# RoboticExplorationLab/TrajectoryOptimization.jl

Hardware: NVIDIA H100
Metric: ilqr_iterations_per_sec (higher is better)
Workload: dtype f64

## Files before the change

trajectoryoptimization.jl_b200/csrc/capi.cu:

```cuda
#include <cmath>
#include <cstdio>
#include <cstring>
#include <string>
#include <vector>

#include "../../include/trajopt_b200.h"
#include "frag_layout.cuh"
#include "kernels.h"

namespace {

std::string g_create_error;

struct Scratch {
    void* ptr = nullptr;
    size_t bytes = 0;
};

}

struct to_handle {
    DevProblem P{};
    int device = 0;
    cudaStream_t stream = nullptr;
// ... 446 lines not shown
    P.ldab = (mn >= 8 && mn <= 16 && mn + mm + 1 <= 20) ? 20 : ((mn + mm + 1) & ~1);
    std::memcpy(P.params, params, sizeof(params));
    set_default_options(P.opt);
    h->t0 = s->t0;
    const int n = mn, m = mm, N = s->N, B = s->B;

    h->h_costs.resize(s->ncost);
    P.all_diag_cost = 1;
    for (int i = 0; i < s->ncost; i++) {
        int rc = build_cost(h, s->costs[i], n, m, h->h_costs[i]);
        if (rc) return bail(rc);
        if (!h->h_costs[i].diag) P.all_diag_cost = 0;
        if (h->h_costs[i].quat || h->h_costs[i].expr) { P.all_diag_cost = 0; P.dense_riccati = 1; }
    }
    P.lie = s->error_state ? 1 : 0; P.qs = 3; P.ne = P.lie ? n - 1 : n;
    if (P.lie) P.dense_riccati = 1;
    {
        bool diag_costs = true;
        for (const auto& c : h->h_costs) if (!c.diag || c.expr || c.quat) diag_costs = false;
        bool diag_cons = true;
        for (int i = 0; i < s->ncon; i++) if (s->cons[i].kind != TO_CON_GOAL && s->cons[i].kind != TO_CON_BOUND) diag_cons = false;
        P.compact = (P.lie && diag_costs && diag_cons && P.ne == 12 && m == 4) ? 1 : 0;
        const char* nf = getenv("TO_NO_FRAG");
        P.frag = (P.compact && !(nf && atoi(nf) != 0)) ? 1 : 0;
    }
    if (P.dense_riccati && !P.compact) h->overlap = false;
    h->h_cost_index.assign(s->cost_index, s->cost_index + N);
    for (int k = 0; k < N; k++)
        if (h->h_cost_index[k] < 0 || h->h_cost_index[k] >= s->ncost) { h->err = "cost_index out of range"; return bail(TO_EINVAL); }
    h->h_cons.resize(s->ncon);
    P.all_diag_con = 1; P.lambda_len = 0;
    for (int i = 0; i < s->ncon; i++) {
        int rc = build_con(h, s->cons[i], n, m, N, h->h_cons[i]);
        if (rc) return bail(rc);
        h->h_cons[i].offset = P.lambda_len;
        P.lambda_len += (h->h_cons[i].last - h->h_cons[i].first + 1) * h->h_cons[i].p;
        if (h->h_cons[i].kind == CON_GOAL) { h->h_cons[i].goff = P.ngoal; P.ngoal += h->h_cons[i].p; }
        if (!h->h_cons[i].diagonal) P.all_diag_con = 0;
    }
    P.ncost = s->ncost; P.ncon = s->ncon;
    P.max_p_knot = 0; P.max_terms_per_z = 0;
    for (int j = 0; j < n + m; j++) {
        int cnt = 0;
        for (const auto& c : h->h_cons) if (c.diagonal) cnt += (c.row_max[j] >= 0) + (c.kind == CON_BOUND && c.row_min[j] >= 0);
        P.max_terms_per_z = std::max(P.max_terms_per_z, cnt);
    }
    P.max_cons_knot = 0;
    for (int k = 1; k <= N; k++) {
        int pk = 0, nk = 0;
        for (const auto& c : h->h_cons) if (k >= c.first && k <= c.last) { pk += c.p; nk++; }
        P.max_p_knot = std::max(P.max_p_knot, pk);
        P.max_cons_knot = std::max(P.max_cons_knot, nk);
    }
    h->h_mu.assign(s->ncon, P.opt.penalty_initial);
    h->h_dt.assign(s->dt, s->dt + (N - 1));
    h->h_dyn = dyn_tab; h->h_dyn_index = dyn_idx;

    int rc = TO_OK;
    double* d_dt = nullptr; int* d_ci = nullptr;
    P.strideX = (size_t)B * N * n; P.strideU = (size_t)B * (N - 1) * m;
#define ALLOC(ptr, count) if (!rc) rc = dalloc(h, &(ptr), (size_t)(count))
    ALLOC(d_dt, N - 1); ALLOC(d_ci, N);
    DevDyn* d_dyn = nullptr; int* d_dyni = nullptr;
    if (!h->h_dyn.empty()) { ALLOC(d_dyn, h->h_dyn.size()); ALLOC(d_dyni, N - 1); }
    ALLOC(h->d_costs, s->ncost); ALLOC(h->d_cons, std::max(1, s->ncon)); ALLOC(h->d_mu, std::max(1, s->ncon));
    ALLOC(P.x0, (size_t)B * n); ALLOC(P.X, TO_NBUF * P.strideX); ALLOC(P.U, TO_NBUF * P.strideU); ALLOC(P.cur, B);
    ALLOC(P.AB, (size_t)B * (N - 1) * n * P.ldab); ALLOC(P.K, (size_t)B * (N - 1) * P.ne * m); ALLOC(P.d, (size_t)B * (N - 1) * m);
    if (P.dense_riccati) {
        const size_t nme = P.ne + m;
        ALLOC(P.ABe, (size_t)B * (N - 1) * P.ne * nme); ALLOC(P.EG, (size_t)B * N * nme); ALLOC(P.EH, (size_t)B * N * nme * nme);
        if (P.compact) ALLOC(P.EC, (size_t)B * N * TO_EC_LEN);
        if (P.frag) ALLOC(P.REC, (size_t)B * N * TO_REC_LEN);
    }
    ALLOC(P.lambda, (size_t)B * std::max(1, P.lambda_len));
    ALLOC(P.rho, B); ALLOC(P.drho, B); ALLOC(P.dV, 2 * (size_t)B); ALLOC(P.J, B); ALLOC(P.Jc, B); ALLOC(P.alpha, B);
    ALLOC(P.bp_status, B); ALLOC(P.ls_iters, B); ALLOC(P.accepted, B); ALLOC(P.acc1, B);
    if (P.frag) { ALLOC(P.late_list, B); ALLOC(P.late_count, 1); }
    ALLOC(h->d_stageX, P.strideX); ALLOC(h->d_stageU, P.strideU); ALLOC(h->d_viol, B); ALLOC(h->d_merit2, 2);
    ALLOC(h->d_work, 1); ALLOC(h->d_err, 1);
    {
        SolveDev& S = h->solve;
        ALLOC(S.state, B); ALLOC(S.status, B); ALLOC(S.iter, B); ALLOC(S.outer, B); ALLOC(S.inner, B); ALLOC(S.dj_zero, B);
        ALLOC(S.J_prev, B); ALLOC(S.dJ, B); ALLOC(S.grad, B); ALLOC(S.cmax, B); ALLOC(S.n_active, 1);
    }
    if (P.frag) { ALLOC(h->d_fragq, frag_queue_ints(B)); ALLOC(h->d_fragpool, frag_pool_doubles(B, N)); ALLOC(h->d_fragerr, 1); ALLOC(h->d_exptab, 1); }
#undef ALLOC
    if (rc) return bail(rc);
    P.exptab = h->d_exptab;
    P.dyn = d_dyn; P.dyn_index = d_dyni;
    P.dt = d_dt; P.cost_index = d_ci; P.costs = h->d_costs; P.cons = h->d_cons; P.mu = h->d_mu; P.viol = h->d_viol;
    cudaStream_t st = h->stream;
    bool okc = true;
    okc &= cudaMemcpyAsync(d_dt, h->h_dt.data(), sizeof(double) * (N - 1), cudaMemcpyHostToDevice, st) == cudaSuccess;
    okc &= cudaMemcpyAsync(d_ci, h->h_cost_index.data(), sizeof(int) * N, cudaMemcpyHostToDevice, st) == cudaSuccess;
    if (d_dyn) {
        okc &= cudaMemcpyAsync(d_dyn, h->h_dyn.data(), sizeof(DevDyn) * h->h_dyn.size(), cudaMemcpyHostToDevice, st) == cudaSuccess;
        okc &= cudaMemcpyAsync(d_dyni, h->h_dyn_index.data(), sizeof(int) * (N - 1), cudaMemcpyHostToDevice, st) == cudaSuccess;
    }
    okc &= cudaMemsetAsync(P.x0, 0, sizeof(double) * B * n, st) == cudaSuccess;
    okc &= cudaMemsetAsync(P.X, 0xFF, sizeof(double) * TO_NBUF * P.strideX, st) == cudaSuccess;
    okc &= cudaMemsetAsync(P.U, 0, sizeof(double) * TO_NBUF * P.strideU, st) == cudaSuccess;
    okc &= cudaMemsetAsync(P.cur, 0, sizeof(int) * B, st) == cudaSuccess;
    okc &= cudaMemsetAsync(P.AB, 0, sizeof(double) * (size_t)B * (N - 1) * n * P.ldab, st) == cudaSuccess;
    okc &= cudaMemsetAsync(P.K, 0, sizeof(double) * (size_t)B * (N - 1) * P.ne * m, st) == cudaSuccess;
    okc &= cudaMemsetAsync(P.d, 0, sizeof(double) * (size_t)B * (N - 1) * m, st) == cudaSuccess;
    okc &= cudaMemsetAsync(P.lambda, 0, sizeof(double) * (size_t)B * std::max(1, P.lambda_len), st) == cudaSuccess;
// ... 900 lines not shown
```

trajectoryoptimization.jl_b200/csrc/common.cuh:

```cuda
#pragma once
#include <cuda_runtime.h>
#include <cstdlib>
#include <stdint.h>

#define TO_MAXN 16
#define TO_MAXM 8
#define TO_MAXNM (TO_MAXN + TO_MAXM)
#define TO_MAXCON 8
#define TO_MAXP 32
#define TO_MAXPV (2 * TO_MAXNM)
#define TO_CON_A 256
#define TO_EXPR_LEN 128
#define TO_EXPR_CONST 64
#define TO_EC_LEN 40
#define TO_NBUF 9

enum { MODEL_DOUBLE_INTEGRATOR = 0, MODEL_CARTPOLE = 1, MODEL_QUADROTOR = 2, MODEL_ACROBOT = 3, MODEL_EXPR = 4 };
enum { CONE_ZERO = 0, CONE_NEGATIVE_ORTHANT = 1, CONE_SECOND_ORDER = 2, CONE_IDENTITY = 3, CONE_POSITIVE_ORTHANT = 4 };
enum { CON_GOAL = 0, CON_BOUND = 1, CON_LINEAR = 2, CON_CIRCLE = 3, CON_SPHERE = 4, CON_NORM = 5, CON_COLLISION = 6, CON_QUATVEC = 7, CON_EXPR = 8 };

struct DevCost {
    int diag, terminal, zeroH, pad;
    double c;
    double Qd[TO_MAXN], Rd[TO_MAXM];
// ... 53 lines not shown
};

struct DevProblem {
    int model, n, m, N, B;
    int ldab;
    int ncost, ncon, lambda_len;
    int all_diag_cost;
    int all_diag_con;
    int max_p_knot;
    int max_terms_per_z;
    int max_cons_knot;
    int lie, ne, qs, dense_riccati;
    int compact, frag;
    double* EC;
    double* REC;
    const ExpTab* exptab;
    const DevDyn* dyn;
    const int* dyn_index;
    double* ABe;
    double* EG;
    double* EH;
    double params[16];
    DevOptions opt;
    const double* dt;
    const DevCost* costs;
    const int* cost_index;
    const DevCon* cons;
    const double* mu;
    double* x0;
    double* X;
    double* U;
    int* cur;
    double* AB;
    double* K;
    double* d;
    double* lambda;
    double* rho;
    double* drho;
    double* dV;
    double* J;
    double* Jc;
    double* viol;
    double* alpha;
    int* bp_status;
    int* ls_iters;
    int* accepted;
    int* acc1;
    int* late_list;
    int* late_count;
    size_t strideX, strideU;
    const int* active;
    const double* qr;
    const double* goal;
    int ngoal, pad_inst;
};

enum { SOLVE_ACTIVE = 0, SOLVE_WAITING = 1, SOLVE_DONE = 2 };
__host__ __device__ inline bool retired(const DevProblem& P, int b) { return P.active != nullptr && P.active[b] != SOLVE_ACTIVE; }

template <bool INST>
__host__ __device__ __forceinline__ const double* inst_q(const DevProblem& P, int b, int cid) {
    if constexpr (INST) { if (P.qr) return P.qr + ((size_t)b * P.ncost + cid) * (P.n + P.m); }
    return P.costs[cid].q;
}
template <bool INST>
__host__ __device__ __forceinline__ const double* inst_r(const DevProblem& P, int b, int cid) {
    if constexpr (INST) { if (P.qr) return P.qr + ((size_t)b * P.ncost + cid) * (P.n + P.m) + P.n; }
    return P.costs[cid].r;
}
template <bool INST>
__host__ __device__ __forceinline__ const double* goal_values(const DevProblem& P, int b, int ci) {
    if constexpr (INST) { if (P.goal) return P.goal + (size_t)b * P.ngoal + P.cons[ci].goff; }
    return P.cons[ci].a;
}

__host__ __device__ inline const double* traj_X(const DevProblem& P, int buf, int b) { return P.X + buf * P.strideX + (size_t)b * P.N * P.n; }
__host__ __device__ inline const double* traj_U(const DevProblem& P, int buf, int b) { return P.U + buf * P.strideU + (size_t)b * (P.N - 1) * P.m; }
__host__ __device__ inline double* traj_Xw(const DevProblem& P, int buf, int b) { return P.X + buf * P.strideX + (size_t)b * P.N * P.n; }
__host__ __device__ inline double* traj_Uw(const DevProblem& P, int buf, int b) { return P.U + buf * P.strideU + (size_t)b * (P.N - 1) * P.m; }

#define TO_MAXDEV 64
inline int current_device_slot() { int d = 0; cudaGetDevice(&d); return (d >= 0 && d < TO_MAXDEV) ? d : 0; }

__host__ __device__ inline void reg_increase(const DevOptions& o, double& rho, double& drho) {
    drho = fmax(drho * o.bp_reg_increase_factor, o.bp_reg_increase_factor);
    rho = fmax(rho * drho, o.bp_reg_min);
}
__host__ __device__ inline void reg_decrease(const DevOptions& o, double& rho, double& drho) {
    drho = fmin(drho / o.bp_reg_increase_factor, 1.0 / o.bp_reg_increase_factor);
    rho = rho * drho * ((rho * drho > o.bp_reg_min) ? 1.0 : 0.0);
}
```

trajectoryoptimization.jl_b200/csrc/forward.cu:

```cuda
#include <cstdlib>
#include "costcon.cuh"
#include "kernels.h"
#include "models.cuh"

namespace {

constexpr int FWD_MAX_COST = 4;
constexpr int FWD_MAX_N = 512;
constexpr int FWD_THREADS = 32;

struct FwdCon {
    int kind, first, last, p, offset;
    unsigned mask_max, mask_min;
    int ubox;
    double mu, inv2mu;
    int row_max[TO_MAXNM], row_min[TO_MAXNM];
    double a[TO_MAXNM], b[TO_MAXNM];
};
struct FwdCost {
    double Qd[TO_MAXN], Rd[TO_MAXM], q[TO_MAXN], r[TO_MAXM], c;
};
struct alignas(16) FwdTab {
    int ncon, ncost_cached, pad0, pad1;
    FwdCon con[TO_MAXCON];
    FwdCost cost[FWD_MAX_COST];
    double dt[FWD_MAX_N];
    int cost_index[FWD_MAX_N];
    int lam_off[FWD_MAX_N][2];
    int lam_cnt[FWD_MAX_N][2];
};

__device__ inline void load_tables(const DevProblem& P, FwdTab& tab) {
    const int t = threadIdx.x, T = blockDim.x;
    if (t == 0) { tab.ncon = P.ncon; tab.ncost_cached = P.ncost <= FWD_MAX_COST ? P.ncost : 0; }
    for (int ci = 0; ci < P.ncon; ci++) {
        const DevCon& c = P.cons[ci];
        FwdCon& f = tab.con[ci];
        if (t == 0) {
            f.kind = c.kind; f.first = c.first; f.last = c.last; f.p = c.p; f.offset = c.offset;
            f.mu = P.mu[ci]; f.inv2mu = 1.0 / (2.0 * P.mu[ci]);
            unsigned mx = 0, mn = 0;
            for (int j = 0; j < TO_MAXNM; j++) { if (c.row_max[j] >= 0) mx |= 1u << j; if (c.row_min[j] >= 0) mn |= 1u << j; }
            f.mask_max = mx; f.mask_min = mn;
            const unsigned ubits = ((1u << P.m) - 1u) << P.n;
            f.ubox = (c.kind == CON_BOUND && mx == ubits && mn == ubits) ? 1 : 0;
        }
        for (int j = t; j < TO_MAXNM; j += T) {
            f.row_max[j] = c.row_max[j]; f.row_min[j] = c.row_min[j];
            f.a[j] = c.a[j]; f.b[j] = c.b[j];
        }
    }
    if (P.ncost <= FWD_MAX_COST)
        for (int ci = 0; ci < P.ncost; ci++) {
            const DevCost& c = P.costs[ci];
            FwdCost& f = tab.cost[ci];
            for (int j = t; j < TO_MAXN; j += T) { f.Qd[j] = c.Qd[j]; f.q[j] = c.q[j]; }
            for (int j = t; j < TO_MAXM; j += T) { f.Rd[j] = c.Rd[j]; f.r[j] = c.r[j]; }
            if (t == 0) f.c = c.c;
        }
    for (int k = t; k < P.N && k < FWD_MAX_N; k += T) {
        tab.dt[k] = (k < P.N - 1) ? P.dt[k] : 0.0; tab.cost_index[k] = P.cost_index[k];
        int ns = 0;
        tab.lam_cnt[k][0] = tab.lam_cnt[k][1] = 0; tab.lam_off[k][0] = tab.lam_off[k][1] = 0;
        for (int ci = 0; ci < P.ncon; ci++) {
            const DevCon& c = P.cons[ci];
            if (k + 1 < c.first || k + 1 > c.last) continue;
            if (ns < 2) { tab.lam_off[k][ns] = c.offset + (k + 1 - c.first) * c.p; tab.lam_cnt[k][ns] = c.p; }
            ns++;
        }
    }
    __syncthreads();
}

__device__ __forceinline__ void cp_async8(double* smem_dst, const double* gsrc) {
    asm volatile("cp.async.ca.shared.global [%0], [%1], 8;" ::"r"((uint32_t)__cvta_generic_to_shared(smem_dst)), "l"(gsrc) : "memory");
}
__device__ __forceinline__ void cp_async16(double* smem_dst, const double* gsrc) {
    asm volatile("cp.async.cg.shared.global [%0], [%1], 16;" ::"r"((uint32_t)__cvta_generic_to_shared(smem_dst)), "l"(gsrc) : "memory");
}
__device__ __forceinline__ void cp_async_commit() { asm volatile("cp.async.commit_group;" ::: "memory"); }
#ifndef TO_FWD_STAGES
#define TO_FWD_STAGES 2
#endif
constexpr int FWD_STAGES = TO_FWD_STAGES;
template <int NPEND> __device__ __forceinline__ void cp_async_wait() { asm volatile("cp.async.wait_group %0;" ::"n"(NPEND) : "memory"); }

template <int n, int m, int IPB, int NE = n>
struct Stage {
    static constexpr int KSLOTS = NE * m;
    static constexpr bool K16 = (KSLOTS % 2) == 0;
    static constexpr int OFF_D = KSLOTS, OFF_U = OFF_D + m, OFF_X = OFF_U + m, OFF_L = OFF_X + n;
    static constexpr int LAM_SLOTS = 2 * (n + m);
    static constexpr int NSLOT = OFF_L + LAM_SLOTS;
    static constexpr int DOUBLES = NSLOT * IPB;
    __device__ static __forceinline__ int kidx(int e, int g) { return K16 ? ((e >> 1) * IPB + g) * 2 + (e & 1) : e * IPB + g; }
    __device__ static __forceinline__ int sidx(int slot, int g) { return slot * IPB + g; }
};

template <int n, int m, int IPB, int G, int NE>
__device__ __forceinline__ void prefetch_knot(double* base, int g, int l, int k, const double* Kg, const double* dg, const double* X,
                                              const double* U, const double* lam_b, const FwdTab& tab, int N) {
    using S = Stage<n, m, IPB, NE>;
    if (k < N - 1) {
        const double* Kk = Kg + (size_t)k * NE * m;
        if (S::K16) {
#pragma unroll
            for (int c = 0; c < (S::KSLOTS / 2 + G - 1) / G; c++) {
                const int cc = c * G + l;
                if (cc < S::KSLOTS / 2) cp_async16(base + S::kidx(2 * cc, g), Kk + 2 * cc);
            }
        } else {
#pragma unroll
            for (int c = 0; c < (S::KSLOTS + G - 1) / G; c++) {
                const int cc = c * G + l;
                if (cc < S::KSLOTS) cp_async8(base + S::kidx(cc, g), Kk + cc);
            }
        }
#pragma unroll
        for (int c = 0; c < (2 * m + n + G - 1) / G; c++) {
            const int s = c * G + l;
            if (s < m) cp_async8(base + S::sidx(S::OFF_D + s, g), dg + (size_t)k * m + s);
            else if (s < 2 * m) cp_async8(base + S::sidx(S::OFF_U + s - m, g), U + (size_t)k * m + (s - m));
            else if (s < 2 * m + n) cp_async8(base + S::sidx(S::OFF_X + s - 2 * m, g), X + (size_t)k * n + (s - 2 * m));
        }
    }
    {
        const int c0 = tab.lam_cnt[k][0], c1 = tab.lam_cnt[k][1];
        const double* l0 = lam_b + tab.lam_off[k][0];
        const double* l1 = lam_b + tab.lam_off[k][1];
        for (int i = l; i < c0; i += G) cp_async8(base + S::sidx(S::OFF_L + i, g), l0 + i);
        for (int i = l; i < c1; i += G) cp_async8(base + S::sidx(S::OFF_L + c0 + i, g), l1 + i);
    }
}

template <int MODEL, int IPB, int G, bool LIE, bool INST>
__device__ __forceinline__ double rollout_fast(const DevProblem& P, const FwdTab& tab, double* stage, int b, int g, int l, unsigned gmask,
                                               double alpha, int cbuf, bool& ok, double& viol) {
    constexpr int n = ModelDims<MODEL>::n, m = ModelDims<MODEL>::m, NE = LIE ? n - 1 : n;
    using S = Stage<n, m, IPB, NE>;
    const int N = P.N, buf = P.cur[b];
    const double* X = traj_X(P, buf, b);
    const double* U = traj_U(P, buf, b);
    double* Xc = traj_Xw(P, cbuf, b);
    double* Uc = traj_Uw(P, cbuf, b);
    const double* Kg = P.K + (size_t)b * (N - 1) * NE * m;
    const double* dg = P.d + (size_t)b * (N - 1) * m;
    const double* lam_b = P.lambda + (size_t)b * P.lambda_len;
    double x[n], u[m], xn[n];
    double J = 0.0;
    ok = true; viol = 0.0;
#pragma unroll
    for (int i = 0; i < n; i++) x[i] = P.x0[(size_t)b * n + i];
    constexpr int D = FWD_STAGES - 1;
#pragma unroll
    for (int j = 0; j < D; j++) {
        if (j < N) prefetch_knot<n, m, IPB, G, NE>(stage + j * S::DOUBLES, g, l, j, Kg, dg, X, U, lam_b, tab, N);
        cp_async_commit();
    }
    int sb = 0, sp = D;
    for (int k = 0; k < N; k++) {
        const bool last = (k == N - 1);
        __syncwarp(gmask);
        if (k + D < N) prefetch_knot<n, m, IPB, G, NE>(stage + sp * S::DOUBLES, g, l, k + D, Kg, dg, X, U, lam_b, tab, N);
        cp_async_commit();
        cp_async_wait<D>();
        __syncwarp(gmask);
        const double* st = stage + sb * S::DOUBLES;
        sb = (sb + 1 == FWD_STAGES) ? 0 : sb + 1; sp = (sp + 1 == FWD_STAGES) ? 0 : sp + 1;
        if (!last) {
#pragma unroll
            for (int a = 0; a < m; a++) u[a] = fma(alpha, st[S::sidx(S::OFF_D + a, g)], st[S::sidx(S::OFF_U + a, g)]);
            double dxe[NE];
            if constexpr (LIE) {
                double xr[n];
#pragma unroll
                for (int i = 0; i < n; i++) xr[i] = st[S::sidx(S::OFF_X + i, g)];
                state_diff(true, n, 3, x, xr, dxe);
            } else {
// ... 64 lines not shown
                double a = 0.0, l2 = 0.0;
                if (c.kind == CON_GOAL) {
                    const unsigned mk = c.mask_max;
                    const double* ga = c.a;
                    if constexpr (INST) ga = goal_values<true>(P, b, ci);
#pragma unroll
                    for (int i = 0; i < n; i++) {
                        if (mk & (1u << i)) {
                            const int row = c.row_max[i];
                            const double lm = st[S::sidx(lo + row, g)];
                            const double cv = x[i] - ga[row];
                            const double lp = fma(-mu, cv, lm);
                            a = fma(lp, lp, a); l2 = fma(lm, lm, l2); viol = fmax(viol, fabs(cv));
                        }
                    }
                } else if (c.ubox) {
#pragma unroll
                    for (int i = 0; i < m; i++) {
                        const double lu = st[S::sidx(lo + i, g)], ll = st[S::sidx(lo + m + i, g)];
                        const double cu = u[i] - c.a[n + i], cl = c.b[n + i] - u[i];
                        const double pu = fmin(0.0, fma(-mu, cu, lu)), pl = fmin(0.0, fma(-mu, cl, ll));
                        a = fma(pu, pu, a); a = fma(pl, pl, a); l2 = fma(lu, lu, l2); l2 = fma(ll, ll, l2);
                        viol = fmax(viol, fmax(cu, cl));
                    }
                } else {
                    const unsigned mx = c.mask_max, mn = c.mask_min;
                    if ((mx | mn) & ((1u << n) - 1u)) {
#pragma unroll
                        for (int i = 0; i < n; i++) {
                            if (mx & (1u << i)) { const double lm = st[S::sidx(lo + c.row_max[i], g)]; const double cv = x[i] - c.a[i]; const double lp = fmin(0.0, fma(-mu, cv, lm)); a = fma(lp, lp, a); l2 = fma(lm, lm, l2); viol = fmax(viol, cv); }
                            if (mn & (1u << i)) { const double lm = st[S::sidx(lo + c.row_min[i], g)]; const double cv = c.b[i] - x[i]; const double lp = fmin(0.0, fma(-mu, cv, lm)); a = fma(lp, lp, a); l2 = fma(lm, lm, l2); viol = fmax(viol, cv); }
                        }
                    }
#pragma unroll
                    for (int i = 0; i < m; i++) {
                        if (mx & (1u << (n + i))) { const double lm = st[S::sidx(lo + c.row_max[n + i], g)]; const double cv = u[i] - c.a[n + i]; const double lp = fmin(0.0, fma(-mu, cv, lm)); a = fma(lp, lp, a); l2 = fma(lm, lm, l2); viol = fmax(viol, cv); }
                        if (mn & (1u << (n + i))) { const double lm = st[S::sidx(lo + c.row_min[n + i], g)]; const double cv = c.b[n + i] - u[i]; const double lp = fmin(0.0, fma(-mu, cv, lm)); a = fma(lp, lp, a); l2 = fma(lm, lm, l2); viol = fmax(viol, cv); }
                    }
                }
                J = fma(a - l2, c.inv2mu, J);
                slot += c.p;
            }
        }
        if (!last) {
            rk4_step<MODEL, double>(model_params<MODEL>(P, k), x, u, tab.dt[k], xn);
#pragma unroll
            for (int i = 0; i < n; i++) { x[i] = xn[i]; if (!(fabs(xn[i]) <= P.opt.max_state_value)) ok = false; }
        }
    }
    cp_async_wait<0>();
    return J;
}

template <int MODEL, bool LIE, bool INST>
__device__ __forceinline__ double rollout_generic(const DevProblem& P, int b, double alpha, int cbuf, bool& ok, double& viol) {
    constexpr int n = ModelDims<MODEL>::n, m = ModelDims<MODEL>::m, NE = LIE ? n - 1 : n;
    const int N = P.N, buf = P.cur[b];
    const double* X = traj_X(P, buf, b);
    const double* U = traj_U(P, buf, b);
    double* Xc = traj_Xw(P, cbuf, b);
    double* Uc = traj_Uw(P, cbuf, b);
    const double* Kg = P.K + (size_t)b * (N - 1) * NE * m;
    const double* dg = P.d + (size_t)b * (N - 1) * m;
    const double* lam_b = P.lambda + (size_t)b * P.lambda_len;
    double x[n], u[m], xn[n];
    double J = 0.0;
    ok = true; viol = 0.0;
#pragma unroll
    for (int i = 0; i < n; i++) x[i] = P.x0[(size_t)b * n + i];
    for (int k = 0; k < N; k++) {
        const bool last = (k == N - 1);
        if (!last) {
#pragma unroll
            for (int a = 0; a < m; a++) u[a] = fma(alpha, dg[(size_t)k * m + a], U[(size_t)k * m + a]);
            double dxe[NE], xr[n];
#pragma unroll
            for (int i = 0; i < n; i++) xr[i] = X[(size_t)k * n + i];
            state_diff(LIE, n, 3, x, xr, dxe);
#pragma unroll
            for (int i = 0; i < NE; i++) {
                const double dx = dxe[i];
#pragma unroll
                for (int a = 0; a < m; a++) u[a] = fma(Kg[(size_t)k * NE * m + i * m + a], dx, u[a]);
            }
#pragma unroll
            for (int a = 0; a < m; a++) if (!(fabs(u[a]) <= P.opt.max_control_value)) ok = false;
        } else {
#pragma unroll
            for (int a = 0; a < m; a++) u[a] = 0.0;
        }
#pragma unroll
        for (int i = 0; i < n; i++) Xc[(size_t)k * n + i] = x[i];
        if (!last) {
#pragma unroll
            for (int a = 0; a < m; a++) Uc[(size_t)k * m + a] = u[a];
        }
        const int cid = P.cost_index[k];
        J += cost_value(P.costs[cid], inst_q<INST>(P, b, cid), inst_r<INST>(P, b, cid), n, m, x, u, !last);
        J += al_knot_penalty<INST>(P, k + 1, x, u, lam_b, viol, b);
        if (!last) {
            rk4_step<MODEL, double>(model_params<MODEL>(P, k), x, u, P.dt[k], xn);
#pragma unroll
            for (int i = 0; i < n; i++) { x[i] = xn[i]; if (!(fabs(xn[i]) <= P.opt.max_state_value)) ok = false; }
            if (!ok) break;
        }
    }
    return J;
}

__device__ __forceinline__ bool ls_accept(const DevProblem& P, double J, double J_prev, double alpha, double dV1, double dV2, bool ok) {
    if (!ok) return false;
    const double expected = -alpha * (dV1 + alpha * dV2);
    const double z = expected > 0.0 ? (J_prev - J) / expected : -1.0;
    return (z > P.opt.ls_lower && z <= P.opt.ls_upper) || (J < J_prev);
}

extern __shared__ __align__(16) unsigned char fwd_smem[];

template <int MODEL, int G, bool FAST, int LANES, bool LIE, bool INST>
__global__ void __launch_bounds__(FWD_THREADS) k_linesearch(const DevProblem P, int trial0, int first_pass, int final_pass) {
    constexpr int n = ModelDims<MODEL>::n, m = ModelDims<MODEL>::m, NE = LIE ? n - 1 : n;
    constexpr int IPB = LANES / G;
    using S = Stage<n, m, IPB, NE>;
    FwdTab* tab = reinterpret_cast<FwdTab*>(fwd_smem);
    double* stage = reinterpret_cast<double*>(fwd_smem + sizeof(FwdTab));
    const int g = (threadIdx.x % LANES) / G, l = threadIdx.x % G;
    int b = blockIdx.x * IPB + g;
    if (!first_pass && P.late_list) b = (b < *P.late_count) ? P.late_list[b] : P.B;
    const unsigned gmask = (G == 32) ? 0xffffffffu : (((1u << G) - 1u) << (g * G));
    const bool valid = b < P.B && threadIdx.x < LANES && !retired(P, b);
    const int status = valid ? P.bp_status[b] : -1;
    const int was_accepted = (valid && !first_pass) ? P.accepted[b] : 0;
    const bool work = valid && status >= 0 && !was_accepted && trial0 <= P.opt.ls_iters;
    const unsigned any = __ballot_sync(0xffffffffu, work);
    if (FAST && any) load_tables(P, *tab);
    if (!valid) return;
    bool accepted = was_accepted != 0;
    if (work) {
        const int trial = trial0 + l;
        const double alpha = ldexp(1.0, -trial);
        const int cbuf = (P.cur[b] + 1 + l) % TO_NBUF;
        bool ok = false;
        double J, viol = 0.0;
        if (FAST) J = rollout_fast<MODEL, IPB, G, LIE, INST>(P, *tab, stage, b, g, l, gmask, alpha, cbuf, ok, viol);
        else J = rollout_generic<MODEL, LIE, INST>(P, b, alpha, cbuf, ok, viol);
        const bool good = (trial <= P.opt.ls_iters) && ls_accept(P, J, P.J[b], alpha, P.dV[2 * b], P.dV[2 * b + 1], ok);
        const unsigned votes = __ballot_sync(gmask, good) & gmask;
        if (votes) {
            const int win = __ffs(votes) - 1 - g * G;
            if (l == win) {
                P.cur[b] = cbuf; P.J[b] = J; P.viol[b] = viol; P.alpha[b] = alpha; P.ls_iters[b] = trial + 1; P.accepted[b] = 1;
            }
            accepted = true;
        }
    }
    if (l == 0 && first_pass) {
        P.acc1[b] = accepted ? 1 : 0;
        if (!accepted && P.late_list) P.late_list[atomicAdd(P.late_count, 1)] = b;
    }
    if (l == 0 && !accepted) {
        if (first_pass) P.accepted[b] = 0;
        if (status < 0) { P.alpha[b] = 0.0; P.ls_iters[b] = 0; }
        else if (final_pass) {
            double rho = P.rho[b], drho = P.drho[b];
            reg_increase(P.opt, rho, drho);
            rho += P.opt.bp_reg_fp;
            P.rho[b] = rho; P.drho[b] = drho;
            P.alpha[b] = 0.0; P.ls_iters[b] = P.opt.ls_iters + 1;
        }
    }
    (void)sizeof(S);
}

template <int MODEL, int G, bool FAST, int LANES, bool LIE = false, bool INST = false>
cudaError_t launch_pass_l(const DevProblem& P, int trial0, int first_pass, int final_pass, cudaStream_t s) {
    constexpr int n = ModelDims<MODEL>::n, m = ModelDims<MODEL>::m, NE = LIE ? n - 1 : n;
    constexpr int IPB = LANES / G;
    const int blocks = (P.B + IPB - 1) / IPB;
    const size_t smem = FAST ? sizeof(FwdTab) + (size_t)FWD_STAGES * Stage<n, m, IPB, NE>::DOUBLES * sizeof(double) : 0;
    auto kern = k_linesearch<MODEL, G, FAST, LANES, LIE, INST>;
    static bool configured[TO_MAXDEV] = {false};
    const int dev = current_device_slot();
    if (!configured[dev] && smem > 48 * 1024) {
        cudaError_t e = cudaFuncSetAttribute(kern, cudaFuncAttributeMaxDynamicSharedMemorySize, (int)smem);
        if (e != cudaSuccess) return e;
    }
    configured[dev] = true;
    kern<<<blocks, FWD_THREADS, smem, s>>>(P, trial0, first_pass, final_pass);
    return cudaGetLastError();
}

template <int MODEL, int G, bool FAST, bool INST>
cudaError_t launch_pass_i(const DevProblem& P, int trial0, int first_pass, int final_pass, cudaStream_t s) {
    const int lanes = first_pass ? 16 : (P.late_list ? 16 : 32);
    if constexpr (MODEL == MODEL_QUADROTOR) {
        if (P.lie) {
            if (G <= 16 && lanes == 16) return launch_pass_l<MODEL, G, FAST, (G <= 16 ? 16 : 32), true, INST>(P, trial0, first_pass, final_pass, s);
            return launch_pass_l<MODEL, G, FAST, 32, true, INST>(P, trial0, first_pass, final_pass, s);
        }
    }
    if (G <= 16 && lanes == 16) return launch_pass_l<MODEL, G, FAST, (G <= 16 ? 16 : 32), false, INST>(P, trial0, first_pass, final_pass, s);
    return launch_pass_l<MODEL, G, FAST, 32, false, INST>(P, trial0, first_pass, final_pass, s);
}

template <int MODEL, int G, bool FAST>
cudaError_t launch_pass(const DevProblem& P, int trial0, int first_pass, int final_pass, cudaStream_t s) {
    if (P.qr) return launch_pass_i<MODEL, G, FAST, true>(P, trial0, first_pass, final_pass, s);
    return launch_pass_i<MODEL, G, FAST, false>(P, trial0, first_pass, final_pass, s);
}

bool fast_path(const DevProblem& P) {
    return P.all_diag_cost && P.all_diag_con && P.N <= FWD_MAX_N && P.max_p_knot <= 2 * (P.n + P.m) && P.max_cons_knot <= 2;
}

}

cudaError_t launch_forward(const DevProblem& P, cudaStream_t s) {
    cudaError_t e = cudaErrorNotSupported;
    const int final_pass = P.opt.ls_iters < 4;
    if (P.late_list) { e = cudaMemsetAsync(P.late_count, 0, sizeof(int), s); if (e != cudaSuccess) return e; e = cudaErrorNotSupported; }
    if (fast_path(P)) { TO_DISPATCH_MODEL(P.model, P.m, (e = launch_pass<MODEL, 4, true>(P, 0, 1, final_pass, s))); }
    else { TO_DISPATCH_MODEL(P.model, P.m, (e = launch_pass<MODEL, 4, false>(P, 0, 1, final_pass, s))); }
    return e;
}

cudaError_t launch_ladder(const DevProblem& P, cudaStream_t s) {
    cudaError_t e = cudaSuccess;
    for (int trial0 = 4; trial0 <= P.opt.ls_iters && e == cudaSuccess; trial0 += 8) {
        const int final_pass = trial0 + 8 > P.opt.ls_iters;
        if (fast_path(P)) { TO_DISPATCH_MODEL(P.model, P.m, (e = launch_pass<MODEL, 8, true>(P, trial0, 0, final_pass, s))); }
        else { TO_DISPATCH_MODEL(P.model, P.m, (e = launch_pass<MODEL, 8, false>(P, trial0, 0, final_pass, s))); }
    }
    return e;
}

cudaError_t launch_accept(const DevProblem& P, cudaStream_t s) { return cudaSuccess; }
```

Before: 2.635 million.

## Add compact line-search rollout path for uniform diagonal cost and box constraints

```diff
diff --git a/profiles/linesearch_ab.py b/profiles/linesearch_ab.py
--- /dev/null
+++ b/profiles/linesearch_ab.py
@@ -0,0 +1,75 @@
+#!/usr/bin/env python3
+import argparse, json, os, subprocess, sys, tempfile
+
+import numpy as np
+
+ROOT = os.path.dirname(os.path.dirname(os.path.abspath(__file__)))
+DEFAULT = os.path.join(ROOT, "trajectoryoptimization.jl_b200", "libtrajopt_b200.so")
+VARIANT = os.path.join(ROOT, "trajectoryoptimization.jl_b200", "variants", "lib_fwd_loop.so")
+
+
+def card():
+    q = subprocess.run(["nvidia-smi", "--query-gpu=name,power.limit,clocks.max.sm", "--format=csv,noheader"], capture_output=True, text=True)
+    return q.stdout.strip().splitlines()[0] if q.returncode == 0 and q.stdout.strip() else "unknown"
+
+
+def bench(lib, workload, dump):
+    env = dict(os.environ, LIBTRAJOPT_B200=lib)
+    out = subprocess.run([sys.executable, os.path.join(ROOT, "bench.py"), "--gpus", "1", "--steps", "20", "--warmup", "3", "--workload", workload,
+                          "--no-cpu-baseline", "--dump-outputs", dump], capture_output=True, text=True, env=env, cwd=ROOT)
+    line = [l for l in out.stdout.splitlines() if l.startswith("{")]
+    if out.returncode or not line:
+        raise SystemExit(f"bench.py failed on {lib}:\n{out.stderr[-2000:]}")
+    d = json.loads(line[-1])
+    ph = d["roofline"]["phase_ms"]
+    return dict(step=d["ms_per_step"], F=ph["forward"], L=ph["ladder"], C1E1=ph["cost_expansion"] + ph["expand"],
+                E2C2=ph["late_expansion"], R=ph["backward"], phases=ph)
+
+
+def main():
+    ap = argparse.ArgumentParser()
+    ap.add_argument("--reps", type=int, default=3)
+    ap.add_argument("--workload", default="quadrotor")
+    ap.add_argument("--out", default=None)
+    ap.add_argument("--lib", action="append", default=[], metavar="NAME=PATH", help="further libraries to alternate with the two")
+    args = ap.parse_args()
+    tmp = tempfile.mkdtemp(prefix="linesearch_ab_")
+    variant = VARIANT
+    if not os.path.exists(variant):
+        subprocess.run(["bash", os.path.join(ROOT, "profiles", "scripts", "build_variant.sh"), "fwd_loop", "forward.cu", "-DTO_FWD_COMPACT=0"],
+                       check=True, env=dict(os.environ, VARIANT_DIR=tmp), stdout=subprocess.DEVNULL)
+        variant = os.path.join(tmp, "lib_fwd_loop.so")
+    print(f"card: {card()}  workload: {args.workload}", flush=True)
+    libs = {"rollout_fast (-DTO_FWD_COMPACT=0)": variant, "rollout_compact (default)": DEFAULT}
+    libs.update(dict(kv.split("=", 1) for kv in args.lib))
+    runs = {name: [] for name in libs}
+    dumps = []
+    for r in range(args.reps):
+        for name, lib in libs.items():
+            d = os.path.join(tmp, f"dump_{len(dumps)}")
+            res = bench(lib, args.workload, d)
+            runs[name].append(res); dumps.append((name, d))
+            print(f"  {name:36s} step {res['step']:.4f}  F {res['F']:.4f}  L {res['L']:.4f}  C1+E1 {res['C1E1']:.4f}  "
+                  f"E2/C2 {res['E2C2']:.4f}  R {res['R']:.4f}", flush=True)
+    ref_name, ref = dumps[0]
+    identical = True
+    for name, d in dumps[1:]:
+        for f in sorted(os.listdir(ref)):
+            a, b = np.load(os.path.join(ref, f)), np.load(os.path.join(d, f))
+            if a.shape != b.shape or not np.array_equal(a.view(np.uint8), b.view(np.uint8)):
+                identical = False
+                print(f"  DUMP DIFFERS: {f} of {name} against {ref_name}")
+    print(f"dumps bit-identical across all {len(dumps)} runs: {identical}")
+    for name, rs in runs.items():
+        rng = lambda k: f"{min(x[k] for x in rs):.3f}-{max(x[k] for x in rs):.3f}"
+        print(f"{name:36s} step {rng('step')}  F {rng('F')}  L {rng('L')}  C1+E1 {rng('C1E1')}  E2/C2 {rng('E2C2')}  R {rng('R')}")
+    fa, fb = runs["rollout_fast (-DTO_FWD_COMPACT=0)"], runs["rollout_compact (default)"]
+    print(f"every default run faster than every variant run: {max(x['step'] for x in fb) < min(x['step'] for x in fa)}")
+    if args.out:
+        with open(args.out, "w") as fh:
+            json.dump(dict(card=card(), runs=runs, identical=identical), fh, indent=1)
+    sys.exit(0 if identical else 1)
+
+
+if __name__ == "__main__":
+    main()
diff --git a/trajectoryoptimization.jl_b200/csrc/capi.cu b/trajectoryoptimization.jl_b200/csrc/capi.cu
--- a/trajectoryoptimization.jl_b200/csrc/capi.cu
+++ b/trajectoryoptimization.jl_b200/csrc/capi.cu
@@ -522,6 +522,21 @@
         P.max_p_knot = std::max(P.max_p_knot, pk);
         P.max_cons_knot = std::max(P.max_cons_knot, nk);
     }
+    {
+        bool cls = N >= 2 && P.all_diag_cost && P.all_diag_con;
+        for (int k = 1; k < N - 1; k++) if (h->h_cost_index[k] != h->h_cost_index[0]) cls = false;
+        int nbox = 0, ngc = 0;
+        for (const auto& c : h->h_cons) {
+            if (c.kind == CON_BOUND) {
+                bool ubox = c.first == 1 && c.last == N - 1 && c.p == 2 * m;
+                for (int j = 0; j < n + m; j++) if ((c.row_max[j] >= 0) != (j >= n) || (c.row_min[j] >= 0) != (j >= n)) ubox = false;
+                cls = cls && ubox; nbox++;
+            } else if (c.kind == CON_GOAL) {
+                cls = cls && c.first == N && c.last == N; ngc++;
+            } else cls = false;
+        }
+        P.fwd_compact = (cls && nbox <= 1 && ngc <= 1) ? 1 : 0;
+    }
     h->h_mu.assign(s->ncon, P.opt.penalty_initial);
     h->h_dt.assign(s->dt, s->dt + (N - 1));
     h->h_dyn = dyn_tab; h->h_dyn_index = dyn_idx;
diff --git a/trajectoryoptimization.jl_b200/csrc/common.cuh b/trajectoryoptimization.jl_b200/csrc/common.cuh
--- a/trajectoryoptimization.jl_b200/csrc/common.cuh
+++ b/trajectoryoptimization.jl_b200/csrc/common.cuh
@@ -129,7 +129,8 @@
     const int* active;
     const double* qr;
     const double* goal;
-    int ngoal, pad_inst;
+    int ngoal;
+    int fwd_compact;
 };
 
 enum { SOLVE_ACTIVE = 0, SOLVE_WAITING = 1, SOLVE_DONE = 2 };
diff --git a/trajectoryoptimization.jl_b200/csrc/forward.cu b/trajectoryoptimization.jl_b200/csrc/forward.cu
--- a/trajectoryoptimization.jl_b200/csrc/forward.cu
+++ b/trajectoryoptimization.jl_b200/csrc/forward.cu
@@ -1,4 +1,5 @@
 #include <cstdlib>
+#include <type_traits>
 #include "costcon.cuh"
 #include "kernels.h"
 #include "models.cuh"
@@ -72,6 +73,50 @@
     __syncthreads();
 }
 
+struct alignas(16) FwdCompactTab {
+    double2 sx[TO_MAXN];
+    double2 su[TO_MAXM];
+    double2 box[TO_MAXM];
+    double sc, mu, inv2mu, pad0;
+    int cid, tcid, box_off, box_p;
+    int goal_ci, goal_off, goal_p, pad1;
+    FwdCost term;
+    FwdCon goal;
+    double dt[FWD_MAX_N];
+};
+
+__device__ inline void load_compact_tables(const DevProblem& P, FwdCompactTab& tab) {
+    const int t = threadIdx.x, T = blockDim.x;
+    const int cid = P.cost_index[0], tcid = P.cost_index[P.N - 1];
+    const DevCost& c = P.costs[cid];
+    const DevCost& ct = P.costs[tcid];
+    for (int j = t; j < TO_MAXN; j += T) { tab.sx[j] = make_double2(c.Qd[j], c.q[j]); tab.term.Qd[j] = ct.Qd[j]; tab.term.q[j] = ct.q[j]; }
+    for (int j = t; j < TO_MAXM; j += T) tab.su[j] = make_double2(c.Rd[j], c.r[j]);
+    if (t == 0) {
+        tab.sc = c.c; tab.term.c = ct.c; tab.cid = cid; tab.tcid = tcid;
+        tab.box_off = tab.box_p = 0; tab.goal_ci = -1; tab.goal_off = tab.goal_p = 0;
+    }
+    for (int ci = 0; ci < P.ncon; ci++) {
+        const DevCon& k = P.cons[ci];
+        if (k.kind == CON_BOUND) {
+            for (int j = t; j < P.m; j += T) tab.box[j] = make_double2(k.a[P.n + j], k.b[P.n + j]);
+            if (t == 0) { tab.box_off = k.offset; tab.box_p = k.p; tab.mu = P.mu[ci]; tab.inv2mu = 1.0 / (2.0 * P.mu[ci]); }
+        } else {
+            FwdCon& f = tab.goal;
+            if (t == 0) {
+                tab.goal_ci = ci; tab.goal_off = k.offset; tab.goal_p = k.p;
+                f.mu = P.mu[ci]; f.inv2mu = 1.0 / (2.0 * P.mu[ci]);
+                unsigned mx = 0;
+                for (int j = 0; j < TO_MAXNM; j++) if (k.row_max[j] >= 0) mx |= 1u << j;
+                f.mask_max = mx;
+            }
+            for (int j = t; j < TO_MAXNM; j += T) { f.row_max[j] = k.row_max[j]; f.a[j] = k.a[j]; }
+        }
+    }
+    for (int k = t; k < P.N - 1; k += T) tab.dt[k] = P.dt[k];
+    __syncthreads();
+}
+
 __device__ __forceinline__ void cp_async8(double* smem_dst, const double* gsrc) {
     asm volatile("cp.async.ca.shared.global [%0], [%1], 8;" ::"r"((uint32_t)__cvta_generic_to_shared(smem_dst)), "l"(gsrc) : "memory");
 }
@@ -83,6 +128,7 @@
 #define TO_FWD_STAGES 2
 #endif
 constexpr int FWD_STAGES = TO_FWD_STAGES;
+constexpr int FWD_OKNOTS = 4;
 template <int NPEND> __device__ __forceinline__ void cp_async_wait() { asm volatile("cp.async.wait_group %0;" ::"n"(NPEND) : "memory"); }
 
 template <int n, int m, int IPB, int NE = n>
@@ -98,8 +144,8 @@
 };
 
 template <int n, int m, int IPB, int G, int NE>
-__device__ __forceinline__ void prefetch_knot(double* base, int g, int l, int k, const double* Kg, const double* dg, const double* X,
-                                              const double* U, const double* lam_b, const FwdTab& tab, int N) {
+__device__ __forceinline__ void prefetch_operands(double* base, int g, int l, int k, const double* Kg, const double* dg, const double* X,
+                                                  const double* U, int N) {
     using S = Stage<n, m, IPB, NE>;
     if (k < N - 1) {
         const double* Kk = Kg + (size_t)k * NE * m;
@@ -124,6 +170,13 @@
             else if (s < 2 * m + n) cp_async8(base + S::sidx(S::OFF_X + s - 2 * m, g), X + (size_t)k * n + (s - 2 * m));
         }
     }
+}
+
+template <int n, int m, int IPB, int G, int NE>
+__device__ __forceinline__ void prefetch_knot(double* base, int g, int l, int k, const double* Kg, const double* dg, const double* X,
+                                              const double* U, const double* lam_b, const FwdTab& tab, int N) {
+    using S = Stage<n, m, IPB, NE>;
+    prefetch_operands<n, m, IPB, G, NE>(base, g, l, k, Kg, dg, X, U, N);
     {
         const int c0 = tab.lam_cnt[k][0], c1 = tab.lam_cnt[k][1];
         const double* l0 = lam_b + tab.lam_off[k][0];
@@ -294,6 +347,171 @@
     return J;
 }
 
+template <int MODEL, int IPB, int G, bool LIE, bool INST>
+__device__ __forceinline__ double rollout_compact(const DevProblem& P, const FwdCompactTab& tab, double* stage, double* ost, int b, int g,
+                                                  int l, unsigned gmask, double alpha, int cbuf, bool& ok, double& viol) {
+    constexpr int n = ModelDims<MODEL>::n, m = ModelDims<MODEL>::m, NE = LIE ? n - 1 : n;
+    using S = Stage<n, m, IPB, NE>;
+    const int N = P.N, buf = P.cur[b];
+    const double* X = traj_X(P, buf, b);
+    const double* U = traj_U(P, buf, b);
+    double* Xc = traj_Xw(P, cbuf, b);
+    const double* Kg = P.K + (size_t)b * (N - 1) * NE * m;
+    const double* dg = P.d + (size_t)b * (N - 1) * m;
+    const double* lam_b = P.lambda + (size_t)b * P.lambda_len;
+    constexpr int OX = FWD_OKNOTS * n, OL = FWD_OKNOTS * (n + m);
+    double* myx = ost + l * OL;
+    double* myu = myx + OX;
+    const double* cq = INST ? inst_q<true>(P, b, tab.cid) : nullptr;
+    const double* cr = INST ? inst_r<true>(P, b, tab.cid) : nullptr;
+    const bool box = tab.box_p != 0;
+    double x[n], u[m];
+    double J = 0.0;
+    ok = true; viol = 0.0;
+#pragma unroll
+    for (int i = 0; i < n; i++) x[i] = P.x0[(size_t)b * n + i];
+    constexpr int D = FWD_STAGES - 1;
+    auto prefetch = [&](double* base, int k) {
+        prefetch_operands<n, m, IPB, G, NE>(base, g, l, k, Kg, dg, X, U, N);
+        const bool stg = k < N - 1;
+        const int cnt = stg ? tab.box_p : tab.goal_p;
+        const double* src = lam_b + (stg ? tab.box_off + k * tab.box_p : tab.goal_off);
+        for (int i = l; i < cnt; i += G) cp_async8(base + S::sidx(S::OFF_L + i, g), src + i);
+    };
+#pragma unroll
+    for (int j = 0; j < D; j++) {
+        if (j < N) prefetch(stage + j * S::DOUBLES, j);
+        cp_async_commit();
+    }
+    int sb = 0, sp = D;
+    auto next_stage = [&](int k) -> const double* {
+        __syncwarp(gmask);
+        if (k + D < N) prefetch(stage + sp * S::DOUBLES, k + D);
+        cp_async_commit();
+        cp_async_wait<D>();
+        __syncwarp(gmask);
+        const double* st = stage + sb * S::DOUBLES;
+        sb = (sb + 1 == FWD_STAGES) ? 0 : sb + 1; sp = (sp + 1 == FWD_STAGES) ? 0 : sp + 1;
+        return st;
+    };
+    auto knot = [&](int k, double* x) {
+        const double* st = next_stage(k);
+#pragma unroll
+        for (int a = 0; a < m; a++) u[a] = fma(alpha, st[S::sidx(S::OFF_D + a, g)], st[S::sidx(S::OFF_U + a, g)]);
+        double dxe[NE];
+        if constexpr (LIE) {
+            double xr[n];
+#pragma unroll
+            for (int i = 0; i < n; i++) xr[i] = st[S::sidx(S::OFF_X + i, g)];
+            state_diff(true, n, 3, x, xr, dxe);
+        } else {
+#pragma unroll
+            for (int i = 0; i < n; i++) dxe[i] = x[i] - st[S::sidx(S::OFF_X + i, g)];
+        }
+#pragma unroll
+        for (int i = 0; i < NE; i++) {
+            const double dx = dxe[i];
+            if (S::K16 && (m % 2 == 0)) {
+#pragma unroll
+                for (int a = 0; a < m; a += 2) {
+                    const double2 kv = *reinterpret_cast<const double2*>(&st[S::kidx(i * m + a, g)]);
+                    u[a] = fma(kv.x, dx, u[a]);
+                    u[a + 1] = fma(kv.y, dx, u[a + 1]);
+                }
+            } else {
+#pragma unroll
+                for (int a = 0; a < m; a++) u[a] = fma(st[S::kidx(i * m + a, g)], dx, u[a]);
+            }
+        }
+#pragma unroll
+        for (int a = 0; a < m; a++) if (!(fabs(u[a]) <= P.opt.max_control_value)) ok = false;
+        const int kk = k % FWD_OKNOTS;
+#pragma unroll
+        for (int i = 0; i < n; i++) myx[kk * n + i] = x[i];
+#pragma unroll
+        for (int a = 0; a < m; a++) myu[kk * m + a] = u[a];
+        if (kk == FWD_OKNOTS - 1 || k == N - 2) {
+            __syncwarp(gmask);
+            const int k0 = k - kk, nx = (kk + 1) * n, nu = (kk + 1) * m;
+            for (int j = 0; j < G; j++) {
+                const int cb = (buf + 1 + j) % TO_NBUF;
+                double* xd = traj_Xw(P, cb, b) + (size_t)k0 * n;
+                double* ud = traj_Uw(P, cb, b) + (size_t)k0 * m;
+                const double* xs = ost + j * OL;
+                for (int e = l; e < nx; e += G) xd[e] = xs[e];
+                for (int e = l; e < nu; e += G) ud[e] = xs[OX + e];
+            }
+        }
+        {
+            double a2 = 0.0, l1 = 0.0;
+#pragma unroll
+            for (int i = 0; i < n; i++) { const double2 c = tab.sx[i]; a2 = fma(c.x * x[i], x[i], a2); l1 = fma(INST ? cq[i] : c.y, x[i], l1); }
+#pragma unroll
+            for (int i = 0; i < m; i++) { const double2 c = tab.su[i]; a2 = fma(c.x * u[i], u[i], a2); l1 = fma(INST ? cr[i] : c.y, u[i], l1); }
+            J += fma(0.5, a2, l1) + tab.sc;
+        }
+        if (box) {
+            const double mu = tab.mu;
+            double a = 0.0, l2 = 0.0;
+#pragma unroll
+            for (int i = 0; i < m; i++) {
+                const double lu = st[S::sidx(S::OFF_L + i, g)], ll = st[S::sidx(S::OFF_L + m + i, g)];
+                const double2 bx = tab.box[i];
+                const double cu = u[i] - bx.x, cl = bx.y - u[i];
+                const double vu = fma(-mu, cu, lu), vl = fma(-mu, cl, ll);
+                const double pu = vu < 0.0 ? vu : 0.0, pl = vl < 0.0 ? vl : 0.0;
+                a = fma(pu, pu, a); a = fma(pl, pl, a); l2 = fma(lu, lu, l2); l2 = fma(ll, ll, l2);
+                const double t = cu > cl ? cu : cl;
+                viol = t > viol ? t : viol;
+            }
+            J = fma(a - l2, tab.inv2mu, J);
+        }
+        if constexpr (MODEL == MODEL_EXPR_42) {
+            double xn[n];
+            rk4_step<MODEL, double>(model_params<MODEL>(P, k), x, u, tab.dt[k], xn);
+#pragma unroll
+            for (int i = 0; i < n; i++) x[i] = xn[i];
+        } else {
+            rk4_step<MODEL, double>(model_params<MODEL>(P, k), x, u, tab.dt[k], x);
+        }
+#pragma unroll
+        for (int i = 0; i < n; i++) if (!(fabs(x[i]) <= P.opt.max_state_value)) ok = false;
+    };
+#pragma unroll 1
+    for (int k = 0; k < N - 1; k++) knot(k, x);
+    {
+        const double* st = next_stage(N - 1);
+#pragma unroll
+        for (int i = 0; i < n; i++) Xc[(size_t)(N - 1) * n + i] = x[i];
+        const double* tq = INST ? inst_q<true>(P, b, tab.tcid) : tab.term.q;
+        double a2 = 0.0, l1 = 0.0;
+#pragma unroll
+        for (int i = 0; i < n; i++) { a2 = fma(tab.term.Qd[i] * x[i], x[i], a2); l1 = fma(tq[i], x[i], l1); }
+        J += fma(0.5, a2, l1) + tab.term.c;
+        if (tab.goal_ci >= 0) {
+            const FwdCon& c = tab.goal;
+            const double mu = c.mu;
+            double a = 0.0, l2 = 0.0;
+            const unsigned mk = c.mask_max;
+            const double* ga = c.a;
+            if constexpr (INST) ga = goal_values<true>(P, b, tab.goal_ci);
+#pragma unroll
+            for (int i = 0; i < n; i++) {
+                if (mk & (1u << i)) {
+                    const int row = c.row_max[i];
+                    const double lm = st[S::sidx(S::OFF_L + row, g)];
+                    const double cv = x[i] - ga[row];
+                    const double lp = fma(-mu, cv, lm);
+                    a = fma(lp, lp, a); l2 = fma(lm, lm, l2); viol = fmax(viol, fabs(cv));
+                }
+            }
+            J = fma(a - l2, c.inv2mu, J);
+        }
+    }
+    cp_async_wait<0>();
+    return J;
+}
+
 template <int MODEL, bool LIE, bool INST>
 __device__ __forceinline__ double rollout_generic(const DevProblem& P, int b, double alpha, int cbuf, bool& ok, double& viol) {
     constexpr int n = ModelDims<MODEL>::n, m = ModelDims<MODEL>::m, NE = LIE ? n - 1 : n;
@@ -359,13 +577,20 @@
 
 extern __shared__ __align__(16) unsigned char fwd_smem[];
 
-template <int MODEL, int G, bool FAST, int LANES, bool LIE, bool INST>
-__global__ void __launch_bounds__(FWD_THREADS) k_linesearch(const DevProblem P, int trial0, int first_pass, int final_pass) {
+enum { FWD_GENERIC = 0, FWD_FAST = 1, FWD_COMPACT = 2 };
+#ifndef TO_FWD_COMPACT
+#define TO_FWD_COMPACT 1
+#endif
+
+template <int MODEL, int G, int PATH, int LANES, bool LIE, bool INST>
+__device__ __forceinline__ void linesearch_pass(const DevProblem& P, int trial0, int first_pass, int final_pass) {
     constexpr int n = ModelDims<MODEL>::n, m = ModelDims<MODEL>::m, NE = LIE ? n - 1 : n;
+    constexpr bool FAST = PATH != FWD_GENERIC;
     constexpr int IPB = LANES / G;
     using S = Stage<n, m, IPB, NE>;
-    FwdTab* tab = reinterpret_cast<FwdTab*>(fwd_smem);
-    double* stage = reinterpret_cast<double*>(fwd_smem + sizeof(FwdTab));
+    using Tab = std::conditional_t<PATH == FWD_COMPACT, FwdCompactTab, FwdTab>;
+    Tab* tab = reinterpret_cast<Tab*>(fwd_smem);
+    double* stage = reinterpret_cast<double*>(fwd_smem + sizeof(Tab));
     const int g = (threadIdx.x % LANES) / G, l = threadIdx.x % G;
     int b = blockIdx.x * IPB + g;
     if (!first_pass && P.late_list) b = (b < *P.late_count) ? P.late_list[b] : P.B;
@@ -375,7 +600,8 @@
     const int was_accepted = (valid && !first_pass) ? P.accepted[b] : 0;
     const bool work = valid && status >= 0 && !was_accepted && trial0 <= P.opt.ls_iters;
     const unsigned any = __ballot_sync(0xffffffffu, work);
-    if (FAST && any) load_tables(P, *tab);
+    if constexpr (PATH == FWD_COMPACT) { if (any) load_compact_tables(P, *tab); }
+    else if (FAST && any) load_tables(P, *tab);
     if (!valid) return;
     bool accepted = was_accepted != 0;
     if (work) {
@@ -384,7 +610,11 @@
         const int cbuf = (P.cur[b] + 1 + l) % TO_NBUF;
         bool ok = false;
         double J, viol = 0.0;
-        if (FAST) J = rollout_fast<MODEL, IPB, G, LIE, INST>(P, *tab, stage, b, g, l, gmask, alpha, cbuf, ok, viol);
+        if constexpr (PATH == FWD_COMPACT) {
+            double* ost = stage + FWD_STAGES * S::DOUBLES + (size_t)g * G * FWD_OKNOTS * (n + m);
+            J = rollout_compact<MODEL, IPB, G, LIE, INST>(P, *tab, stage, ost, b, g, l, gmask, alpha, cbuf, ok, viol);
+        }
+        else if (FAST) J = rollout_fast<MODEL, IPB, G, LIE, INST>(P, *tab, stage, b, g, l, gmask, alpha, cbuf, ok, viol);
         else J = rollout_generic<MODEL, LIE, INST>(P, b, alpha, cbuf, ok, viol);
         const bool good = (trial <= P.opt.ls_iters) && ls_accept(P, J, P.J[b], alpha, P.dV[2 * b], P.dV[2 * b + 1], ok);
         const unsigned votes = __ballot_sync(gmask, good) & gmask;
@@ -414,13 +644,28 @@
     (void)sizeof(S);
 }
 
-template <int MODEL, int G, bool FAST, int LANES, bool LIE = false, bool INST = false>
+template <int MODEL, int G, bool FAST, int LANES, bool LIE, bool INST>
+__global__ void __launch_bounds__(FWD_THREADS) k_linesearch(const DevProblem P, int trial0, int first_pass, int final_pass) {
+    linesearch_pass<MODEL, G, FAST ? FWD_FAST : FWD_GENERIC, LANES, LIE, INST>(P, trial0, first_pass, final_pass);
+}
+
+template <int MODEL, int G, int LANES, bool LIE, bool INST>
+__global__ void __launch_bounds__(FWD_THREADS) k_linesearch_compact(const DevProblem P, int trial0, int first_pass, int final_pass) {
+    linesearch_pass<MODEL, G, FWD_COMPACT, LANES, LIE, INST>(P, trial0, first_pass, final_pass);
+}
+
+template <int MODEL, int G, int PATH, int LANES, bool LIE = false, bool INST = false>
 cudaError_t launch_pass_l(const DevProblem& P, int trial0, int first_pass, int final_pass, cudaStream_t s) {
     constexpr int n = ModelDims<MODEL>::n, m = ModelDims<MODEL>::m, NE = LIE ? n - 1 : n;
     constexpr int IPB = LANES / G;
     const int blocks = (P.B + IPB - 1) / IPB;
-    const size_t smem = FAST ? sizeof(FwdTab) + (size_t)FWD_STAGES * Stage<n, m, IPB, NE>::DOUBLES * sizeof(double) : 0;
-    auto kern = k_linesearch<MODEL, G, FAST, LANES, LIE, INST>;
+    const size_t tab = PATH == FWD_COMPACT ? sizeof(FwdCompactTab) : sizeof(FwdTab);
+    const size_t ost = PATH == FWD_COMPACT ? (size_t)LANES * FWD_OKNOTS * (n + m) * sizeof(double) : 0;
+    const size_t smem = PATH != FWD_GENERIC ? tab + (size_t)FWD_STAGES * Stage<n, m, IPB, NE>::DOUBLES * sizeof(double) + ost : 0;
+    auto kern = [] {
+        if constexpr (PATH == FWD_COMPACT) return k_linesearch_compact<MODEL, G, LANES, LIE, INST>;
+        else return k_linesearch<MODEL, G, PATH == FWD_FAST, LANES, LIE, INST>;
+    }();
     static bool configured[TO_MAXDEV] = {false};
     const int dev = current_device_slot();
     if (!configured[dev] && smem > 48 * 1024) {
@@ -432,27 +677,36 @@
     return cudaGetLastError();
 }
 
-template <int MODEL, int G, bool FAST, bool INST>
+template <int MODEL, int G, int PATH, bool INST>
 cudaError_t launch_pass_i(const DevProblem& P, int trial0, int first_pass, int final_pass, cudaStream_t s) {
     const int lanes = first_pass ? 16 : (P.late_list ? 16 : 32);
     if constexpr (MODEL == MODEL_QUADROTOR) {
         if (P.lie) {
-            if (G <= 16 && lanes == 16) return launch_pass_l<MODEL, G, FAST, (G <= 16 ? 16 : 32), true, INST>(P, trial0, first_pass, final_pass, s);
-            return launch_pass_l<MODEL, G, FAST, 32, true, INST>(P, trial0, first_pass, final_pass, s);
-        }
-    }
-    if (G <= 16 && lanes == 16) return launch_pass_l<MODEL, G, FAST, (G <= 16 ? 16 : 32), false, INST>(P, trial0, first_pass, final_pass, s);
-    return launch_pass_l<MODEL, G, FAST, 32, false, INST>(P, trial0, first_pass, final_pass, s);
-}
-
-template <int MODEL, int G, bool FAST>
+            if (G <= 16 && lanes == 16) return launch_pass_l<MODEL, G, PATH, (G <= 16 ? 16 : 32), true, INST>(P, trial0, first_pass, final_pass, s);
+            return launch_pass_l<MODEL, G, PATH, 32, true, INST>(P, trial0, first_pass, final_pass, s);
+        }
+    }
+    if (G <= 16 && lanes == 16) return launch_pass_l<MODEL, G, PATH, (G <= 16 ? 16 : 32), false, INST>(P, trial0, first_pass, final_pass, s);
+    return launch_pass_l<MODEL, G, PATH, 32, false, INST>(P, trial0, first_pass, final_pass, s);
+}
+
+template <int MODEL, int G, int PATH>
 cudaError_t launch_pass(const DevProblem& P, int trial0, int first_pass, int final_pass, cudaStream_t s) {
-    if (P.qr) return launch_pass_i<MODEL, G, FAST, true>(P, trial0, first_pass, final_pass, s);
-    return launch_pass_i<MODEL, G, FAST, false>(P, trial0, first_pass, final_pass, s);
+    if (P.qr) return launch_pass_i<MODEL, G, PATH, true>(P, trial0, first_pass, final_pass, s);
+    return launch_pass_i<MODEL, G, PATH, false>(P, trial0, first_pass, final_pass, s);
 }
 
 bool fast_path(const DevProblem& P) {
     return P.all_diag_cost && P.all_diag_con && P.N <= FWD_MAX_N && P.max_p_knot <= 2 * (P.n + P.m) && P.max_cons_knot <= 2;
+}
+
+bool compact_path(const DevProblem& P) { return TO_FWD_COMPACT && fast_path(P) && P.fwd_compact && P.ncost <= FWD_MAX_COST; }
+
+template <int MODEL, int G>
+cudaError_t launch_any(const DevProblem& P, int trial0, int first_pass, int final_pass, cudaStream_t s) {
+    if constexpr (TO_FWD_COMPACT) { if (compact_path(P)) return launch_pass<MODEL, G, FWD_COMPACT>(P, trial0, first_pass, final_pass, s); }
+    if (fast_path(P)) return launch_pass<MODEL, G, FWD_FAST>(P, trial0, first_pass, final_pass, s);
+    return launch_pass<MODEL, G, FWD_GENERIC>(P, trial0, first_pass, final_pass, s);
 }
 
 }
@@ -461,8 +715,7 @@
     cudaError_t e = cudaErrorNotSupported;
     const int final_pass = P.opt.ls_iters < 4;
     if (P.late_list) { e = cudaMemsetAsync(P.late_count, 0, sizeof(int), s); if (e != cudaSuccess) return e; e = cudaErrorNotSupported; }
-    if (fast_path(P)) { TO_DISPATCH_MODEL(P.model, P.m, (e = launch_pass<MODEL, 4, true>(P, 0, 1, final_pass, s))); }
-    else { TO_DISPATCH_MODEL(P.model, P.m, (e = launch_pass<MODEL, 4, false>(P, 0, 1, final_pass, s))); }
+    TO_DISPATCH_MODEL(P.model, P.m, (e = launch_any<MODEL, 4>(P, 0, 1, final_pass, s)));
     return e;
 }
 
@@ -470,8 +723,7 @@
     cudaError_t e = cudaSuccess;
     for (int trial0 = 4; trial0 <= P.opt.ls_iters && e == cudaSuccess; trial0 += 8) {
         const int final_pass = trial0 + 8 > P.opt.ls_iters;
-        if (fast_path(P)) { TO_DISPATCH_MODEL(P.model, P.m, (e = launch_pass<MODEL, 8, true>(P, trial0, 0, final_pass, s))); }
-        else { TO_DISPATCH_MODEL(P.model, P.m, (e = launch_pass<MODEL, 8, false>(P, trial0, 0, final_pass, s))); }
+        TO_DISPATCH_MODEL(P.model, P.m, (e = launch_any<MODEL, 8>(P, trial0, 0, final_pass, s)));
     }
     return e;
 }
```

Measured after the change: 2.891 million (median of 6 runs). 1.1x the previous value.
